# dsilvestro/LiteRate

Measured on AMD Instinct MI355X. Metric: RJMCMC iters/sec x lineages (lineage-log-lik evals/s, summed over chains), higher is better.
Workload: dtype f64

## Files before the change

### literate_amd/_hip.py

```python
import ctypes as C
import os

from .build import LIB

c_i32, c_i64, c_f64, c_vp = C.c_int32, C.c_int64, C.c_double, C.c_void_p

LR_ERR_NULL, LR_ERR_SIZE, LR_ERR_MODEL, LR_ERR_WORKSPACE, LR_ERR_T0, LR_ERR_STATE, LR_ERR_ORDER = -1, -2, -3, -4, -5, -6, -7
ERRORS = {-1: "LR_ERR_NULL", -2: "LR_ERR_SIZE", -3: "LR_ERR_MODEL", -4: "LR_ERR_WORKSPACE", -5: "LR_ERR_T0",
          -6: "LR_ERR_STATE", -7: "LR_ERR_ORDER (lineages must be sorted by birth time for the persistent engines)"}

LR_KMAX, LR_ROW, LR_MAX_BINS = 32, 64, 4094
LR_WARN_KCAP = 2
LR_STATE_ROWS, LR_ISTATE_ROWS = 9, 5
LR_TRACE_HEAD = 13
LR_TRACE_W = LR_TRACE_HEAD + 2 * (2 * LR_KMAX - 1)
LR_SIMBATCH_GROUPS, LR_SIMBATCH_LDS_SLOTS = 512, 16384
LR_SHIFT_PRIOR_KCAP, LR_SHIFT_PRIOR_BLOCKS = 64, 768
LR_ESS_LDS_ROWS = 16384
ROW_L, ROW_M, ROW_TL, ROW_TM, ROW_PL, ROW_PM, ROW_PTL, ROW_PTM, ROW_SCALARS = range(9)
(S_LIKA, S_PRIORA, S_PRIORPOIA, S_GRATE_L, S_GRATE_M, S_POI, S_HASTING, S_PRIOR_P, S_PRIORPOI_P, S_CONST_P,
 S_CONST_A, S_LIK_P, S_LOG_G0, S_LOG_G1, S_LOG_POI) = range(15)
IROW_EL, IROW_EM, IROW_PEL, IROW_PEM, IROW_SCALARS = range(5)
(I_KL, I_KM, I_PKL, I_PKM, I_GIBBS, I_INVALID, I_IT_LO, I_IT_HI, I_ACCEPTED, I_MOVE, I_NEXT_LO, I_NEXT_HI,
 I_SLOT) = range(13)


class McmcConfig(C.Structure):
    _fields_ = [("n_lineages", c_i64), ("n_bins", c_i32), ("n_chains", c_i32), ("model", c_i32),
                ("const_rates", c_i32), ("const_death_rate", c_i32), ("use_rate_HP", c_i32), ("s_freq", c_i32),
                ("n_trace_slots", c_i32), ("poisson_HP", c_f64), ("update_fraction", c_f64), ("t0", c_f64),
# ... 60 lines not shown
    "lr_curve_summary": (c_i32, [c_vp, c_i32, c_i32, c_i32, c_i32, c_i32, c_i32, c_i32, c_vp, c_i32, c_f64, c_i32, c_vp,
                                 c_vp, c_i64, c_vp]),
    "lr_mcmc_query_layout": (c_i32, [C.POINTER(McmcConfig), C.POINTER(McmcLayout)]),
    "lr_mcmc_create": (c_i32, [C.POINTER(McmcConfig), c_vp, c_vp, c_vp, c_vp, c_i64, C.POINTER(c_vp)]),
    "lr_mcmc_init": (c_i32, [c_vp, c_vp, c_vp, c_vp, c_vp, c_vp, c_vp, c_i32, c_vp]),
    "lr_mcmc_steps": (c_i32, [c_vp, c_i64, c_vp]),
    "lr_mcmc_time_scan": (c_i32, [c_vp, c_i32, C.POINTER(C.c_float), c_vp]),
    "lr_mcmc_time_steps": (c_i32, [c_vp, c_i64, C.POINTER(C.c_float), c_vp]),
    "lr_mcmc_restore": (c_i32, [c_vp, c_vp]),
    "lr_mcmc_describe": (c_i32, [c_vp, C.c_char_p, c_i32]),
    "lr_mcmc_status": (c_i32, [c_vp, C.POINTER(c_i32), c_vp]),
    "lr_mcmc_warnings": (c_i32, [c_vp, C.POINTER(c_i32), c_vp]),
    "lr_mcmc_destroy": (c_i32, [c_vp]),
    "lr_debug_draws": (c_i32, [C.c_uint64, c_i64, c_vp, c_vp, c_vp, c_vp, c_vp, c_i32, c_vp, c_vp]),
    "lr_debug_stream2": (c_i32, [c_vp, c_vp, c_i64, c_vp, c_vp]),
}

_lib = None


class HipLibraryError(RuntimeError):
    pass


def load():
    global _lib
    if _lib is not None:
        return _lib
    if not os.path.exists(LIB):
        raise HipLibraryError("libliterate_hip.so not found at %s - run `python -m literate_amd.build` "
# ... 38 lines not shown
```

### literate_amd/build.py

```python
import json
import os
import shutil
import subprocess
from concurrent.futures import ThreadPoolExecutor

HERE = os.path.dirname(os.path.abspath(__file__))
CSRC = os.path.join(HERE, "csrc")
LIB = os.path.join(CSRC, "libliterate_hip.so")
BUILD_INFO = os.path.join(CSRC, "libliterate_hip.build.json")
OBJ_DIR = os.path.join(CSRC, "_build")
SOURCES = ["lr_stats.hip", "lr_loglik.hip", "lr_mcmc.hip", "lr_spec.hip", "lr_stream.hip", "lr_packscan.hip", "lr_pack.hip", "lr_sim.hip", "lr_simbatch.hip", "lr_format.hip", "lr_summary.hip", "lr_prior.hip", "lr_ess.hip", "lr_curves.hip", "lr_waic.hip", "lr_loo.hip"]
HEADERS = ["lr_device.h", "lr_math.h", "lr_chain.h", "lr_dd.h", "lr_scan.h", "lr_step.h", "lr_spec.h", "lr_engine.h", "lr_internal.h",
           os.path.join("..", "..", "include", "literate_hip.h")]
TU_FLAGS = {"lr_spec.hip": os.environ.get("LR_SPEC_FLAGS", "-mllvm -disable-machine-licm").split(),
            "lr_mcmc.hip": os.environ.get("LR_MCMC_FLAGS", "-mllvm -disable-machine-licm").split(),
            "lr_stream.hip": os.environ.get("LR_STREAM_FLAGS", "-mllvm -disable-machine-licm").split()}
ASYNC_UNITS = {"lr_mcmc.hip": 60, "lr_spec.hip": 0, "lr_packscan.hip": 16}


def _stale():
    if not os.path.exists(LIB):
        return True
    t = os.path.getmtime(LIB)
    return any(os.path.getmtime(os.path.join(CSRC, f)) > t for f in SOURCES + HEADERS)


# ... 72 lines not shown
```

### literate_amd/csrc/lr_engine.h

```cpp
#pragma once
#include "lr_internal.h"
#include "lr_scan.h"
#include "lr_step.h"

#define LR_MAX_PARTS 4
struct lr_part {
    int base, count, hA;
    bool pipelined;
    hipStream_t stream;
    hipEvent_t done;
    hipGraphExec_t graph_exec;
    int graph_units;
};

struct lr_p4_shares {
    int delta[16];
    int n_slots;
    int help_trips;
};

struct lr_engine {
    lr_mcmc_config cfg;
    lr_mcmc_layout lay;
    lr_scan_plan plan;
// ... 14 lines not shown
    hipEvent_t fork;
    hipEvent_t ev0, ev1;
};


#define LR_P4_MAX_GIVE 64
#define LR_IDX_SPARE ((LR_P4_MAX_GIVE + 2) * 1024)
#define LR_MAX_RUNS (1ll << 20)

static inline long long lr_groups_alloc(long long n_lineages) {
    const long long runs = n_lineages < LR_MAX_RUNS ? n_lineages : LR_MAX_RUNS;
    return (n_lineages + LR_SLOTS - 1) / LR_SLOTS + runs + LR_IDX_SPARE;
}

#define LR_P4_CARRY_BYTES 512

#define LR_H_WIDE 520

#ifndef LR_SPEC_THREADS
#define LR_SPEC_THREADS 768
#endif
#ifndef LR_SPEC_THREADS_SINGLE
#define LR_SPEC_THREADS_SINGLE 768
#endif
#ifndef LR_SPEC_SCAN_UNROLL
#define LR_SPEC_SCAN_UNROLL 1
#endif
#ifndef LR_SPEC_SCAN_PRIO
#define LR_SPEC_SCAN_PRIO 2
#endif
// ... 43 lines not shown
```

### literate_amd/csrc/lr_mcmc.hip

```cpp
#include <cmath>
#include <cstdio>
#include <cstdlib>
#include <new>

#include "lr_chain.h"
#include "lr_dd.h"
#include "lr_engine.h"
#include "lr_internal.h"
#include "lr_scan.h"
#include "lr_step.h"

__global__ __launch_bounds__(LR_WAVE) void lr_rj_propose_score_kernel(
    const double* __restrict__ rates, const double* __restrict__ times, const int* __restrict__ K, int kmax,
    const int* __restrict__ move, const int* __restrict__ index, const double* __restrict__ draws, double mult_d,
    double* __restrict__ out_rates, double* __restrict__ out_times, int* __restrict__ out_K,
    double* __restrict__ out_score) {
    const int c = blockIdx.x, lane = threadIdx.x;
    int k = K[c];
    double R = (lane < k) ? rates[(size_t)c * kmax + lane] : 0.0;
    double T = (lane <= k) ? times[(size_t)c * (kmax + 1) + lane] : 0.0;
    const double* dr = draws + (size_t)c * 2 * kmax;
    const int mv = move[c];
    double score = 0.0;
    if (mv == 0) {
// ... 146 lines not shown
    lr_persist_scan<H, GENERAL>(reinterpret_cast<const char*>(tab), pk, g0, g1 - g0, tid, 256, &acc0, &acc1);
    const double s0 = lr_wave_sum(acc0), s1 = lr_wave_sum(acc1);
    if (lane == 0) red[wave][0] = s0, red[wave][1] = s1;
    __syncthreads();
    if (tid < 2 && 2 * pair + tid < n_chains)
        partials[(size_t)(2 * pair + tid) * lr_tile_stride(tiles) + tile] = ((red[0][tid] + red[1][tid]) + red[2][tid]) + red[3][tid];
}

typedef __attribute__((address_space(3))) double lr_lds_f64;
typedef __attribute__((address_space(3))) int lr_lds_i32;
template <int PB, int ES, bool PRE = false, int SAMPLER = -1, bool HAND = false>
__device__ __forceinline__ void lr_persist_step_body(const __attribute__((address_space(3))) lr_step_args* a3, int c, int lane,
                                                     __attribute__((address_space(3))) lr_seg_scratch* scratch3,
                                                     lr_lds_f64* st_f64, lr_lds_i32* st_i32, double lik, lr_lds_f64* table3,
                                                     lr_lds_f64* br3 ,
                                                     const lr_draw_slot* draws = nullptr ,
                                                     lr_table_hand* hand = nullptr, int hand_epoch = 0) {
    constexpr int table_es = ES;
    const lr_step_args& a = *(const lr_step_args*)a3;
    const double* br_lds = (const double*)br3;
    LR_SSTAMP(0);
    lr_chain_regs st;
    lr_chain_load(st, (double*)st_f64, (int*)st_i32, lane);
    if (SAMPLER == 1 || (SAMPLER == -1 && a.cfg.sampler != 0))
        lr_dd_step_core<true>(st, a, 0, c, lane, lik, reinterpret_cast<double2*>((double*)table3), table_es, br_lds);
    else if (PRE) {
        lr_rj_draws pre;
        lr_draws_load(draws, pre, lane);
        lr_chain_step_core<true, PB, HAND>(st, a, 0, c, lane, (lr_seg_scratch*)scratch3, lik, reinterpret_cast<double2*>((double*)table3),
                                           table_es, br_lds, br_lds + LR_H_WIDE, &pre, hand, hand_epoch);
    } else
        lr_chain_step_core<true, PB>(st, a, 0, c, lane, (lr_seg_scratch*)scratch3, lik, reinterpret_cast<double2*>((double*)table3),
                                     table_es, br_lds, br_lds + LR_H_WIDE);
    if (HAND) lr_chain_store_handed(st, (double*)st_f64, (int*)st_i32, lane);
    else lr_chain_store(st, (double*)st_f64, (int*)st_i32, lane);
    LR_SSTAMP(8);
}

template <int NA>
__device__ __forceinline__ void lr_p4_leave_sums(double2 (*part)[LR_WAVE], int* arrived, double* out, int slot, int lane,
                                                 int& scans_done, double s0, double s1) {
    part[slot][lane] = make_double2(s0, s1);
    int prev = 0;
// ... 15 lines not shown

template <int PB, int ES>
__device__ __attribute__((noinline)) void lr_persist_step(const __attribute__((address_space(3))) lr_step_args* a3, int c, int lane,
                                                          __attribute__((address_space(3))) lr_seg_scratch* scratch3,
                                                          lr_lds_f64* st_f64, lr_lds_i32* st_i32, double lik, lr_lds_f64* table3,
                                                          lr_lds_f64* br3) {
    lr_persist_step_body<PB, ES>(a3, c, lane, scratch3, st_f64, st_i32, lik, table3, br3);
}

template <int PB, int ES, int NW, int SAMPLER, bool HELP>
__device__ __attribute__((noinline)) void lr_persist4_steppers(const __attribute__((address_space(3))) lr_step_args* a3, int c0,
                                                               int n_chains, int wave, int lane,
                                                               __attribute__((address_space(3))) lr_seg_scratch* scratch3,
                                                               lr_lds_f64* st_f64, lr_lds_i32* st_i32, lr_lds_f64* red,
                                                               lr_lds_f64* tab, int tab_doubles, lr_lds_f64* br3, long long n_iters,
                                                               const lr_draw_slot* draws ,
                                                               lr_table_hand* hands ) {
    static_assert(!HELP || (ES == 2 && SAMPLER == 0), "helper waves: RJ sampler at unit resolution");
    for (long long iter = 0; iter < n_iters; ++iter) {
#pragma unroll 1
        for (int ph = 0; ph < 2; ++ph) {
#ifdef LR_DIAG
            const unsigned long long dq0 = wall_clock64();
#endif
            const int c = c0 + 2 * ph + wave;
            if (c < n_chains) {
                double lik = 0.0;
#pragma unroll
                for (int w2 = 2; w2 < (ES == 2  ? 3 : NW); ++w2) lik += red[(ph * NW + w2) * 2 + wave];
                lr_persist_step_body<PB, ES, ES == 2  && SAMPLER == 0, SAMPLER, HELP>(
                    a3, c, lane, scratch3, st_f64 + (2 * ph + wave) * (LR_STATE_ROWS * LR_ROW),
                    st_i32 + (2 * ph + wave) * (LR_ISTATE_ROWS * LR_ROW), lik, tab + ph * tab_doubles + wave, br3,
                    draws + (2 * ph + wave), HELP ? hands + wave : nullptr, (int)((2 * iter + ph + 1) & 0x3fffffff));
            }
#ifdef LR_DIAG
            const unsigned long long dq1 = wall_clock64();
#endif
            __syncthreads();
#ifdef LR_DIAG
            if (lane == 0 && blockIdx.x < 64) {
                atomicAdd(&lr_diag_step[16384 + (blockIdx.x * 16 + wave) * 4 + 0], dq1 - dq0);
                atomicAdd(&lr_diag_step[16384 + (blockIdx.x * 16 + wave) * 4 + 1], wall_clock64() - dq1);
            }
#endif
        }
    }
}

// ... 131 lines not shown
}

#ifndef LR_P4_THREADS
#define LR_P4_THREADS 1024
#endif
#ifdef LR_DIAG
#define LR_PSTAMP(k) if (threadIdx.x == 0 && blockIdx.x < 64) lr_diag_step[28672 + blockIdx.x * 8 + (k)] = wall_clock64()
#else
#define LR_PSTAMP(k)
#endif

template <int H, bool GENERAL, bool PARAM ,
          bool HELP = false>
__global__ __launch_bounds__(LR_P4_THREADS, LR_P4_THREADS / 256) void lr_persist4_kernel(const lr_step_args* __restrict__ ap ,
                                                                       lr_packed_lineages pk, long long n8,
                                                                       lr_p4_shares sh, long long n_iters, char* carry_all) {
    static_assert(!HELP || (!GENERAL && !PARAM), "helper waves: RJ sampler at unit resolution");
    const lr_step_args& a = *ap;
    LR_PSTAMP(0);
    constexpr int NW = LR_P4_THREADS / LR_WAVE;
    constexpr int W0 = HELP ? 4 : 2;
    constexpr int NS = NW - W0;
    constexpr int LR_P4_SCANNERS = NS * LR_WAVE;
    constexpr int ENT = GENERAL ? 2 : 1;
    constexpr int ES = GENERAL ? 6 * H : 2;
    __shared__ double2 tab[2][LR_UNIT_PLANES * H];
    __shared__ double red[2][NW][2];
    constexpr bool LAST_SUMS = !GENERAL;
    __shared__ double2 part[LAST_SUMS ? NW - 2 : 1][LR_WAVE];
    __shared__ int arrived;
    __shared__ lr_table_hand hands[2];
    __shared__ lr_seg_scratch scratch[2];
    __shared__ double st_f64[4][LR_STATE_ROWS * LR_ROW];
    __shared__ int st_i32[4][LR_ISTATE_ROWS * LR_ROW];
    __shared__ lr_step_args a_lds;
    __shared__ double br_lds[2][LR_H_WIDE];
    __shared__ lr_draw_slot draws_s[4];
    lr_draw_slot* const draws = draws_s;
    const int tid = threadIdx.x, lane = tid & (LR_WAVE - 1), wave = tid / LR_WAVE;
    if (tid < (int)(sizeof(lr_step_args) / 4)) reinterpret_cast<int*>(&a_lds)[tid] = reinterpret_cast<const int*>(ap)[tid];
    for (int b = tid; b < LR_H_WIDE; b += blockDim.x) {
        const bool in = b < ap->cfg.n_bins;
        br_lds[0][b] = (in && ap->br_length) ? ap->br_length[b] : 0.0;
        br_lds[1][b] = in ? ap->log_br[b] : 0.0;
    }
    constexpr bool draw_ahead = !GENERAL && !PARAM;
    auto draw_duty = [&](int pr) {
        const int q = wave - W0, k = q & 1, ch = 2 * pr + k;
        if (!draw_ahead || q < 0 || q >= (HELP ? 2 : 4) || (int)(blockIdx.x * 4) + ch >= ap->cfg.n_chains) return;
        const int* I = st_i32[ch] + LR_IROW_SCALARS * LR_ROW;
        const unsigned long long it = ((unsigned long long)(unsigned int)I[LR_I_IT_HI] << 32 | (unsigned int)I[LR_I_IT_LO]) + 1ull;
        lr_draw_slot* slot = &draws[ch];
        if (HELP) lr_spec_draw_both(a_lds, (int)(blockIdx.x * 4) + ch, lane, it, slot);
        else lr_spec_draw_part(a_lds, (int)(blockIdx.x * 4) + ch, lane, it, slot, q >> 1);
    };
    auto help_duty = [&](int ph, int epoch) {
        const int k = wave - 2;
        const int ch = 2 * ph + k;
        if ((int)(blockIdx.x * 4) + ch >= ap->cfg.n_chains) return;
        lr_table_hand* hand = &hands[k];
#ifdef LR_DIAG
        const unsigned long long dh0 = wall_clock64();
#endif
        while (__hip_atomic_load(&hand->epoch, __ATOMIC_RELAXED, __HIP_MEMORY_SCOPE_WORKGROUP) != epoch) __builtin_amdgcn_s_sleep(1);
        asm volatile("" ::: "memory");
#ifdef LR_DIAG
        if (lane == 0 && blockIdx.x < 64) atomicAdd(&lr_diag_step[16384 + (blockIdx.x * 16 + wave) * 4 + 2], wall_clock64() - dh0);
#endif
        const lr_seg_scratch* sc = &scratch[k];
        const int eL = lane <= LR_KMAX ? sc->edge[0][lane] : 0, eM = lane <= LR_KMAX ? sc->edge[1][lane] : 0;
// ... 15 lines not shown
            lr_p4_leave_sums<NA>(part, &arrived, &red[pr][2][0], wave >= W0 ? wave - W0 : NS + wave - 2, lane, scans_done, s0, s1);
        } else {
            s0 = lr_wave_sum(s0), s1 = lr_wave_sum(s1);
            if (lane == 0) red[pr][wave][0] = s0, red[pr][wave][1] = s1;
        }
    };
    const int c0 = blockIdx.x * 4;
    const int C = a.cfg.n_chains;
    if (wave < 4 && c0 + wave < C) {
        const int c = c0 + wave;
        const double* S = a.state_f64 + (size_t)c * LR_STATE_ROWS * LR_ROW;
        const int* I = a.state_i32 + (size_t)c * LR_ISTATE_ROWS * LR_ROW;
        for (int r = 0; r < LR_STATE_ROWS; ++r) st_f64[wave][r * LR_ROW + lane] = S[r * LR_ROW + lane];
        for (int r = 0; r < LR_ISTATE_ROWS; ++r) st_i32[wave][r * LR_ROW + lane] = I[r * LR_ROW + lane];
    }
    double2* g0 = lr_chain_table(a, c0);
    double2* g1 = lr_chain_table(a, c0 + 2);
    for (int i = tid; i < 2 * H * ENT; i += LR_P4_THREADS) {
        const int e = GENERAL ? lr_pairgen_lds_entry(i, H) : i;
        tab[0][e] = g0[i], tab[1][e] = g1[i];
    }
    __syncthreads();
    LR_PSTAMP(1);
    if (GENERAL) {
        lr_pair_planes_block_general(tab[0], H, a.cfg.n_bins, tid, LR_P4_THREADS);
        lr_pair_planes_block_general(tab[1], H, a.cfg.n_bins, tid, LR_P4_THREADS);
    } else {
        lr_pair_planes_block(tab[0], H, a.cfg.n_bins, tid, LR_P4_THREADS);
        lr_pair_planes_block(tab[1], H, a.cfg.n_bins, tid, LR_P4_THREADS);
    }
// ... 6 lines not shown
    const int k_tot = (int)((n8 - nh_ + LR_P4_SCANNERS - 1) / LR_P4_SCANNERS);
    const int k_mine = k_tot + (scanner ? sh.delta[wave - W0] : 0);
    bool any_shift = false;
#pragma unroll
    for (int q = 0; q < NS; ++q) any_shift |= sh.delta[q] != 0;
    const long long nh = HELP ? (long long)sh.help_trips * (2 * LR_WAVE) : 0;
    const long long n8w = any_shift ? (long long)k_mine * LR_P4_SCANNERS : n8 - nh;
    auto help_scan = [&](int pr) {
        double s0 = 0.0, s1 = 0.0;
        if (nh > 0) lr_persist_scan<H, GENERAL, 1, false, false>(reinterpret_cast<const char*>(tab[pr]), pk, 0, nh, tid - 2 * LR_WAVE, 2 * LR_WAVE, &s0, &s1);
        leave_sums(pr, s0, s1);
    };
    static_assert(2 * NW * 8 + 4 <= LR_P4_CARRY_BYTES, "");
    char* carry = carry_all ? carry_all + (size_t)blockIdx.x * LR_P4_CARRY_BYTES : nullptr;
    const bool carried = carry && *reinterpret_cast<const int*>(carry + 2 * NW * 8) == 1;
    auto prologue_draws = [&]() { draw_duty(0); };
    if (carried) {
        if (tid < 2 * NW) (&red[0][0][0])[tid] = reinterpret_cast<const double*>(carry)[tid];
        if (scanner) prologue_draws();
    } else if (scanner) {
        double s0 = 0.0, s1 = 0.0;
        lr_scan_tail tail;
        lr_persist_scan<H, GENERAL, 1, false, true>(reinterpret_cast<const char*>(tab[0]), pk, nh, n8w, sid, LR_P4_SCANNERS, &s0, &s1, nullptr, &tail);
        leave_sums(0, s0, s1);
        lr_scan_drain(tail);
        prologue_draws();
    }
    if (helper && !carried) help_scan(0);
    __syncthreads();
    LR_PSTAMP(3);
    if (helper) {
        for (long long iter = 0; iter < n_iters; ++iter) {
#pragma unroll 1
            for (int ph = 0; ph < 2; ++ph) {
#ifdef LR_DIAG
                const unsigned long long dq0 = wall_clock64();
#endif
                help_scan(1 - ph);
                help_duty(ph, (int)((2 * iter + ph + 1) & 0x3fffffff));
#ifdef LR_DIAG
                const unsigned long long dq1 = wall_clock64();
#endif
                __syncthreads();
#ifdef LR_DIAG
                if (lane == 0 && blockIdx.x < 64) {
                    atomicAdd(&lr_diag_step[16384 + (blockIdx.x * 16 + wave) * 4 + 0], dq1 - dq0);
                    atomicAdd(&lr_diag_step[16384 + (blockIdx.x * 16 + wave) * 4 + 1], wall_clock64() - dq1);
                }
#endif
            }
        }
    } else if (!scanner)
        lr_persist4_steppers<(H <= 264 ? lr_bins_per_lane(H) : 0), ES, NW, PARAM ? 1 : 0, HELP>(
            (const __attribute__((address_space(3))) lr_step_args*)&a_lds, c0, C, wave, lane,
            (__attribute__((address_space(3))) lr_seg_scratch*)&scratch[wave], (lr_lds_f64*)&st_f64[0][0], (lr_lds_i32*)&st_i32[0][0],
            (lr_lds_f64*)&red[0][0][0], (lr_lds_f64*)reinterpret_cast<double*>(tab[0]), 2 * LR_UNIT_PLANES * H,
            (lr_lds_f64*)&br_lds[0][0], n_iters, &draws[0], &hands[0]);
    else
    for (long long iter = 0; iter < n_iters; ++iter) {
#pragma unroll
        for (int ph = 0; ph < 2; ++ph) {
#ifdef LR_DIAG
            const unsigned long long dq0 = wall_clock64();
#endif
            {
                double s0 = 0.0, s1 = 0.0;
                lr_scan_tail tail;
                lr_persist_scan<H, GENERAL, 1, false, true>(reinterpret_cast<const char*>(tab[1 - ph]), pk, nh, n8w, sid, LR_P4_SCANNERS, &s0, &s1, nullptr, &tail);
                leave_sums(1 - ph, s0, s1);
                lr_scan_drain(tail);
                draw_duty(1 - ph);
            }
#ifdef LR_DIAG
            const unsigned long long dq1 = wall_clock64();
#endif
            __syncthreads();
#ifdef LR_DIAG
            if (lane == 0 && blockIdx.x < 64) {
                atomicAdd(&lr_diag_step[16384 + (blockIdx.x * 16 + wave) * 4 + 0], dq1 - dq0);
                atomicAdd(&lr_diag_step[16384 + (blockIdx.x * 16 + wave) * 4 + 1], wall_clock64() - dq1);
            }
#endif
        }
    }
    LR_PSTAMP(4);
    if (wave < 4 && c0 + wave < C) {
// ... 399 lines not shown
    out->pack_tmp = o, o += lr_align_up64(lr_pack_tmp_bytes(cfg->n_lineages), 256);
    out->args_blob = o, o += 1024;
    out->tables = o, o += lr_align_up64((long long)lr_align_up64(C, p.cb < 2 ? 2 : p.cb) * p.tab_stride * 16, 256);
    out->partials = o, o += lr_align_up64((long long)lr_tile_stride(p.tiles) * C * 8, 256);
    out->trace = o, o += lr_align_up64((long long)cfg->n_trace_slots * C * LR_TRACE_W * 8, 256);
    int team_k = 0, team_cpb = 0;
    out->persistent = lr_persist_variant(cfg, p, &team_k, &team_cpb);
    out->spec_chains_per_team = team_cpb;
    {
        int base[LR_MAX_PARTS + 1], hA[LR_MAX_PARTS];
        bool pipelined[LR_MAX_PARTS];
        const bool packed = lr_packscan_planned(cfg, p);
        const int parts = lr_partition(cfg->n_chains, p.cb, lr_fused_supported(p), base, hA, pipelined, lr_packed_mode(cfg, p));
        out->packed_scan = (out->persistent == 0 && packed) ? 1 : 0;
        out->streaming = (out->persistent == 0 && !out->packed_scan && parts == 1 && !pipelined[0] && lr_stream_eligible(cfg, p)) ? 1 : 0;
        out->reserved3 = 0;
    }
    if (p.unit == LR_TAB_PAIRGEN && out->persistent == 0 && !lr_packscan_planned(cfg, p)) return LR_ERR_STATE;
    out->team_blocks = team_k;
    out->table_mode = p.unit;
    out->status = o, o += 256;
    out->xchg = o, o += (team_k > 1) ? lr_align_up64(2ll * C * LR_TEAM_MAX * LR_SPEC_GRANULES * 8, 256)
                                     : (out->persistent == 2 ? lr_align_up64((C + 3) / 4 * LR_P4_CARRY_BYTES, 256)
                                        : (out->streaming ? LR_STREAM_SYNC_BYTES + lr_align_up64((long long)lr_align_up64(C, p.cb < 2 ? 2 : p.cb) * p.tab_stride * 16, 256) : 0));
    out->total_bytes = o;
    out->table_stride = p.tab_stride;
    out->tiles = p.tiles;
    out->chains_per_block = p.cb;
    out->trace_width = LR_TRACE_W;
    {
        int base[LR_MAX_PARTS + 1], hA[LR_MAX_PARTS];
        bool pipelined[LR_MAX_PARTS];
        out->n_parts = lr_partition(cfg->n_chains, p.cb, lr_fused_supported(p), base, hA, pipelined, lr_packed_mode(cfg, p));
        out->pipelined = pipelined[0] ? 1 : 0;
    }
    {
        static const int wide_env = lr_env_int("LR_PERSIST_WIDE", -1);
        const bool wide = wide_env >= 0 ? wide_env != 0 : ((cfg->n_chains + 1) / 2 <= 256 && cfg->n_lineages >= 20000);
        out->reserved1 = out->persistent == 3 ? (team_cpb == 1 ? LR_SPEC_THREADS_SINGLE : LR_SPEC_THREADS) : (out->persistent == 2 ? 1024 : (out->persistent == 1 ? (wide ? 1024 : 512) : 0));
// ... 327 lines not shown
    hipStream_t stream = (hipStream_t)stream_;
    const lr_step_args a = lr_make_args(e);
    if (e->persistent) {
        const uint4* idx8 = (const uint4*)(e->ws + e->lay.lineage_idx);
        const bool general = e->plan.unit == LR_TAB_PAIRGEN;
        lr_packed_lineages pk;
        pk.idx8 = idx8, pk.frac = general ? (const uint4*)(e->ws + e->lay.lineage_frac) : nullptr, pk.fstride = e->n8_alloc;
        if (e->n8 <= 0) return LR_ERR_STATE;
        const lr_step_args* ap = (const lr_step_args*)(e->ws + e->lay.args_blob);
        const int blocks = (e->cfg.n_chains + 1) / 2;
        const bool p4 = e->lay.persistent == 2;
        const bool param = e->cfg.sampler != 0;
        static const int prio = lr_env_int("LR_PERSIST_PRIO", 12);
        const bool wide = e->lay.reserved1 == 1024;
        if (e->lay.persistent == 3) return lr_launch_spec(e, a, pk, n_iters, stream);
        for (int64_t done = 0; done < n_iters;) {
            const int64_t n = (n_iters - done > 4096) ? 4096 : n_iters - done;
        static const int carry_env = lr_env_int("LR_P4_CARRY", 1);
        char* p4_carry = (p4 && carry_env) ? e->ws + e->lay.xchg : nullptr;
#define LR_P_LAUNCH(HH)                                                                                                       \
    if (p4) {                                                                                                                 \
        const dim3 g4((e->cfg.n_chains + 3) / 4), b4(LR_P4_THREADS);                                                          \
        if (general && param) hipLaunchKernelGGL((lr_persist4_kernel<HH, true, true>), g4, b4, 0, stream, ap, pk, e->n8, e->p4, (long long)n, p4_carry);   \
        else if (general) hipLaunchKernelGGL((lr_persist4_kernel<HH, true, false>), g4, b4, 0, stream, ap, pk, e->n8, e->p4, (long long)n, p4_carry);      \
        else if (param) hipLaunchKernelGGL((lr_persist4_kernel<HH, false, true>), g4, b4, 0, stream, ap, pk, e->n8, e->p4, (long long)n, p4_carry);        \
        else if (e->p4_help)                                                 \
            hipLaunchKernelGGL((lr_persist4_kernel<(HH <= 264 ? HH : 264), false, false, true>), g4, b4, 0, stream, ap, pk, e->n8, e->p4, (long long)n, p4_carry); \
        else hipLaunchKernelGGL((lr_persist4_kernel<HH, false, false>), g4, b4, 0, stream, ap, pk, e->n8, e->p4, (long long)n, p4_carry);                  \
    } else if (wide) {                                                                                                        \
        hipLaunchKernelGGL((lr_persist_kernel<HH, 1024>), dim3(blocks), dim3(1024), 0, stream, ap, idx8, e->n8, e->p4, (long long)n, 0); \
    } else {                                                                                                                  \
        hipLaunchKernelGGL((lr_persist_kernel<HH, 512>), dim3(blocks), dim3(512), 0, stream, ap, idx8, e->n8, e->p4, (long long)n, prio); \
    }
            switch (e->plan.H) {
                case 40: LR_P_LAUNCH(40); break;
                case 72: LR_P_LAUNCH(72); break;
                case 136: LR_P_LAUNCH(136); break;
                case 264: LR_P_LAUNCH(264); break;
                default: LR_P_LAUNCH(LR_H_WIDE); break;
            }
#undef LR_P_LAUNCH
            const int rc = (int)hipGetLastError();
            if (rc) return rc;
// ... 127 lines not shown
```

### literate_amd/csrc/lr_step.h

```cpp
#pragma once
#include "lr_chain.h"
#include "lr_dd.h"
#include "lr_internal.h"
#include "lr_scan.h"

struct lr_step_args {
    lr_mcmc_config cfg;
    double* state_f64;
    int* state_i32;
    const double* log_br;
    double2* tables;
    const double* partials;
    double* trace;
    const double* br_length;
    double log_T;
    double mult_l;
    const double* dd_consts;
    int tab_stride, n_cls, tiles, H, unit, cb;
    unsigned int* warn;
};

__device__ __forceinline__ double2* lr_chain_table(const lr_step_args& a, int c) {
    if (!a.unit) return a.tables + (size_t)c * a.tab_stride;
    if (a.unit == LR_TAB_PAIRGEN)
// ... 494 lines not shown
    double beta = 0.0;
    if (!(r_a < 0.8) && r_a < 0.999 && cfg.const_rates == 0 && q_b > 0.5) {
        double ga, gb;
        lr_wave_gamma2(rng, it, LR_P_BETA_A, LR_SHAPE_BETA_RJ, LR_P_BETA_B, LR_SHAPE_BETA_RJ, lane, &ga, &gb);
        beta = ga / (ga + gb);
    }
    double so = lr_bcast(lu, LR_UD_LANE);
    so = (lane == 1) ? r_a : so;
    so = (lane == 2) ? lr_bcast(u.b, LR_UD_LANE + 1) : so;
    so = (lane == 3) ? lr_bcast(u.a, LR_UD_LANE + 2) : so;
    so = (lane == 4) ? q_b : so;
    so = (lane == 5) ? lr_bcast(u.a, LR_UD_LANE + 3) : so;
    so = (lane == 6) ? lr_bcast(u.b, LR_UD_LANE + 3) : so;
    so = (lane == 7) ? beta : so;
    if (lane < 8) out->sc[lane] = so;
}

struct lr_table_hand {
    int epoch;
    int KL, KM;
    int reuse;
    int noop;
    int out_idx, base_idx;
    int pad_;
    double par[8];
};

template <bool LDS_CONSTS = false, int PB = 0, int CS = 2, bool PAIR_PLANES = true, bool HAND = false>
__device__ __forceinline__ void lr_propose_rj(const lr_step_args& a, int c, int lane, lr_seg_scratch* scratch_p,
                                              uint64_t it, lr_rj_state& s, lr_rj_prop& p, double2* table,
// ... 529 lines not shown
```

### literate_amd/engine.py

```python
import ctypes as C
import hashlib
import os
from collections import namedtuple

import numpy as np

from . import _hip, ops


class ChainEngine:
    def __init__(self, ts, te, n_chains, model=0, seed=1, const_rates=0, const_death_rate=0, use_rate_HP=1,
                 poisson_HP=0.0, update_fraction=0.75, s_freq=1000, n_trace_slots=0, chain_offset=0,
                 device=None, stats=None, sort_lineages=True, unit_resolution=None, engine="auto", dd=None, team=0,
                 chains_per_team=0):
        torch = _hip.require_gpu()
        self.lib = _hip.load()
        self.device = torch.device(device or "cuda")
        ts_d = ops._dev(ts, torch.float64, self.device)
        te_d = ops._dev(te, torch.float64, self.device)
        if sort_lineages:
            o1 = torch.sort(te_d, stable=True).indices
            o2 = torch.sort(torch.floor(ts_d[o1]), stable=True).indices
            order = o1[o2]
            ts_d, te_d = ts_d[order].contiguous(), te_d[order].contiguous()
# ... 213 lines not shown
    _CFG_KEYS = ("n_lineages", "n_bins", "n_chains", "model", "const_rates", "const_death_rate", "use_rate_HP",
                 "s_freq", "n_trace_slots", "poisson_HP", "update_fraction", "t0", "start_time", "end_time", "seed",
                 "chain_offset", "unit_resolution", "frac_birth", "frac_death", "sampler", "m_birth", "m_death",
                 "dd_present", "dd_init_death", "engine_mode")

    def _signature(self):
        sig = {k: repr(getattr(self.cfg, k)) for k in self._CFG_KEYS}
        sig.update({"layout_" + f: repr(getattr(self.layout, f)) for f, _ in self.layout._fields_})
        sig["data_sha1"] = self._data_hash
        sig["format"] = "2: state in .npz (head, tail), trace rows in .npz.trace"
        return sig

    def _trace_span(self):
        return int(self.layout.trace), int(self.layout.status)

    def checkpoint_begin(self):
        import torch
        t0, t1 = self._trace_span()
        with torch.cuda.device(self.device):
            head, tail = self.workspace[:t0].clone(), self.workspace[t1:].clone()
            ev = torch.cuda.Event()
            ev.record()
        return dict(head=head, tail=tail, ev=ev, iterations=int(self.iterations), samples=int(self.samples_done()))

    def checkpoint_write(self, ticket, path):
        import torch
        path = str(path)
        if not path.endswith(".npz"):
            path += ".npz"
        side = getattr(self, "_ckpt_stream", None)
        if side is None:
            side = self._ckpt_stream = torch.cuda.Stream(device=self.device)
        row_bytes = self.n_chains * _hip.LR_TRACE_W * 8
        s1 = ticket["samples"]
        sidecar = path + ".trace"
# ... 33 lines not shown
        ticket = self.checkpoint_begin()
        self.check_status()
        self.checkpoint_write(ticket, path)

    def load(self, path):
        import torch
        path = str(path)
        with np.load(path) as z:
            saved = dict(zip([str(k) for k in z["sig_keys"]], [str(v) for v in z["sig_vals"]]))
            mine = self._signature()
            bad = [k for k in mine if k not in saved or mine[k] != saved[k]]
            if bad or len(saved) != len(mine):
                raise ValueError("checkpoint was written by a different configuration: " + ", ".join(bad))
            t0, t1 = self._trace_span()
            head, tail = torch.from_numpy(z["head"]), torch.from_numpy(z["tail"])
            if head.numel() != t0 or tail.numel() != self.workspace.numel() - t1:
                raise ValueError("checkpoint workspace size differs")
            n_rows = int(z["n_trace_rows"])
            row_bytes = self.n_chains * _hip.LR_TRACE_W * 8
            if n_rows > 0:
                sidecar = path + ".trace"
                if not os.path.exists(sidecar) or os.path.getsize(sidecar) < n_rows * row_bytes:
                    raise ValueError("checkpoint trace file %s is missing or shorter than the %d rows the checkpoint holds" % (sidecar, n_rows))
                rows = np.fromfile(sidecar, dtype=np.uint8, count=n_rows * row_bytes)
                self.workspace[t0:t0 + n_rows * row_bytes].copy_(torch.from_numpy(rows).to(self.device))
            self.workspace[:t0].copy_(head.to(self.device))
            self.workspace[t1:].copy_(tail.to(self.device))
            self.iterations = int(z["iterations"])
        self._ckpt_saved = {path: n_rows}
        _hip.check(_hip.launch(self.lib.lr_mcmc_restore, self.device, self.handle), "lr_mcmc_restore")

    def close(self):
        if getattr(self, "handle", None) is not None:
            self.lib.lr_mcmc_destroy(self.handle)
            self.handle = None

    def __del__(self):
        try:
            self.close()
        except Exception:
            pass

# ... 119 lines not shown
```

Measured before the change: 16100 billion.

## Pre-draw RJ random numbers in a separate kernel before persistent4 chunks

Moves the per-iteration RJ draws out of the persistent4 kernel, where scanner/helper waves produced them into shared slots, into a separate predraw kernel. That kernel fills a global record buffer for a chunk of iterations and all chains. The persistent kernel then loads each chain's next record with a nontemporal vector load one phase ahead, which takes RNG work off the critical step path. The cost is extra workspace (up to about 1 GiB), an extra launch per chunk, and global memory traffic.

```diff
diff --git a/literate_amd/_hip.py b/literate_amd/_hip.py
--- a/literate_amd/_hip.py
+++ b/literate_amd/_hip.py
@@ -14,6 +14,7 @@
 LR_STATE_ROWS, LR_ISTATE_ROWS = 9, 5
 LR_TRACE_HEAD = 13
 LR_TRACE_W = LR_TRACE_HEAD + 2 * (2 * LR_KMAX - 1)
+LR_REC_DOUBLES = 128
 LR_SIMBATCH_GROUPS, LR_SIMBATCH_LDS_SLOTS = 512, 16384
 LR_SHIFT_PRIOR_KCAP, LR_SHIFT_PRIOR_BLOCKS = 64, 768
 LR_ESS_LDS_ROWS = 16384
@@ -104,6 +105,7 @@
     "lr_mcmc_destroy": (c_i32, [c_vp]),
     "lr_debug_draws": (c_i32, [C.c_uint64, c_i64, c_vp, c_vp, c_vp, c_vp, c_vp, c_i32, c_vp, c_vp]),
     "lr_debug_stream2": (c_i32, [c_vp, c_vp, c_i64, c_vp, c_vp]),
+    "lr_debug_rj_draws": (c_i32, [C.POINTER(McmcConfig), c_i32, c_i32, C.c_uint64, c_i32, c_vp, c_vp, c_vp]),
 }
 
 _lib = None
diff --git a/literate_amd/build.py b/literate_amd/build.py
--- a/literate_amd/build.py
+++ b/literate_amd/build.py
@@ -9,7 +9,7 @@
 LIB = os.path.join(CSRC, "libliterate_hip.so")
 BUILD_INFO = os.path.join(CSRC, "libliterate_hip.build.json")
 OBJ_DIR = os.path.join(CSRC, "_build")
-SOURCES = ["lr_stats.hip", "lr_loglik.hip", "lr_mcmc.hip", "lr_spec.hip", "lr_stream.hip", "lr_packscan.hip", "lr_pack.hip", "lr_sim.hip", "lr_simbatch.hip", "lr_format.hip", "lr_summary.hip", "lr_prior.hip", "lr_ess.hip", "lr_curves.hip", "lr_waic.hip", "lr_loo.hip"]
+SOURCES = ["lr_stats.hip", "lr_loglik.hip", "lr_mcmc.hip", "lr_predraw.hip", "lr_spec.hip", "lr_stream.hip", "lr_packscan.hip", "lr_pack.hip", "lr_sim.hip", "lr_simbatch.hip", "lr_format.hip", "lr_summary.hip", "lr_prior.hip", "lr_ess.hip", "lr_curves.hip", "lr_waic.hip", "lr_loo.hip"]
 HEADERS = ["lr_device.h", "lr_math.h", "lr_chain.h", "lr_dd.h", "lr_scan.h", "lr_step.h", "lr_spec.h", "lr_engine.h", "lr_internal.h",
            os.path.join("..", "..", "include", "literate_hip.h")]
 TU_FLAGS = {"lr_spec.hip": os.environ.get("LR_SPEC_FLAGS", "-mllvm -disable-machine-licm").split(),
diff --git a/literate_amd/csrc/lr_engine.h b/literate_amd/csrc/lr_engine.h
--- a/literate_amd/csrc/lr_engine.h
+++ b/literate_amd/csrc/lr_engine.h
@@ -52,6 +52,24 @@
 }
 
 #define LR_P4_CARRY_BYTES 512
+
+static inline int lr_p4_rec_chains(int n_chains) { return (n_chains + 3) / 4 * 4; }
+static inline int lr_p4_draw_chunk_default(int persistent, int table_mode, const lr_mcmc_config* cfg) {
+    if (persistent != 2 || table_mode == LR_TAB_PAIRGEN || cfg->sampler != 0) return 0;
+    const long long b = (1ll << 30) / ((long long)lr_p4_rec_chains(cfg->n_chains) * (LR_REC_DOUBLES * 8));
+    return b > 4096 ? 4096 : (b < 1 ? 1 : (int)b);
+}
+static inline int lr_p4_draw_chunk(const lr_engine* e) {
+    static const char* env = getenv("LR_P4_DRAW_CHUNK");
+    const int v = env ? atoi(env) : 0;
+    return (v >= 1 && v < e->lay.reserved3) ? v : e->lay.reserved3;
+}
+static inline long long lr_p4_recs_offset(const lr_engine* e) {
+    return e->lay.xchg + lr_align_up64((long long)(e->cfg.n_chains + 3) / 4 * LR_P4_CARRY_BYTES, 256);
+}
+int lr_launch_predraw(uint64_t seed, int64_t chain_offset, int const_rates, double mult_l, const int* state_i32,
+                      unsigned long long it_first, int chain_first, int n_chains, int n_iters, int rec_cq, double* recs,
+                      hipStream_t stream);
 
 #define LR_H_WIDE 520
 
diff --git a/literate_amd/csrc/lr_mcmc.hip b/literate_amd/csrc/lr_mcmc.hip
--- a/literate_amd/csrc/lr_mcmc.hip
+++ b/literate_amd/csrc/lr_mcmc.hip
@@ -184,7 +184,7 @@
                                                      __attribute__((address_space(3))) lr_seg_scratch* scratch3,
                                                      lr_lds_f64* st_f64, lr_lds_i32* st_i32, double lik, lr_lds_f64* table3,
                                                      lr_lds_f64* br3 ,
-                                                     const lr_draw_slot* draws = nullptr ,
+                                                     lr_f64x2 rec = lr_f64x2{0.0, 0.0} ,
                                                      lr_table_hand* hand = nullptr, int hand_epoch = 0) {
     constexpr int table_es = ES;
     const lr_step_args& a = *(const lr_step_args*)a3;
@@ -196,7 +196,7 @@
         lr_dd_step_core<true>(st, a, 0, c, lane, lik, reinterpret_cast<double2*>((double*)table3), table_es, br_lds);
     else if (PRE) {
         lr_rj_draws pre;
-        lr_draws_load(draws, pre, lane);
+        lr_draws_from_rec(rec, pre, lane);
         lr_chain_step_core<true, PB, HAND>(st, a, 0, c, lane, (lr_seg_scratch*)scratch3, lik, reinterpret_cast<double2*>((double*)table3),
                                            table_es, br_lds, br_lds + LR_H_WIDE, &pre, hand, hand_epoch);
     } else
@@ -242,9 +242,11 @@
                                                                __attribute__((address_space(3))) lr_seg_scratch* scratch3,
                                                                lr_lds_f64* st_f64, lr_lds_i32* st_i32, lr_lds_f64* red,
                                                                lr_lds_f64* tab, int tab_doubles, lr_lds_f64* br3, long long n_iters,
-                                                               const lr_draw_slot* draws ,
+                                                               const double* recs, int rec_cq, lr_f64x2 rec0,
                                                                lr_table_hand* hands ) {
     static_assert(!HELP || (ES == 2 && SAMPLER == 0), "helper waves: RJ sampler at unit resolution");
+    constexpr bool PRE = ES == 2  && SAMPLER == 0;
+    lr_f64x2 rec = rec0;
     for (long long iter = 0; iter < n_iters; ++iter) {
 #pragma unroll 1
         for (int ph = 0; ph < 2; ++ph) {
@@ -256,10 +258,14 @@
                 double lik = 0.0;
 #pragma unroll
                 for (int w2 = 2; w2 < (ES == 2  ? 3 : NW); ++w2) lik += red[(ph * NW + w2) * 2 + wave];
-                lr_persist_step_body<PB, ES, ES == 2  && SAMPLER == 0, SAMPLER, HELP>(
+                lr_persist_step_body<PB, ES, PRE, SAMPLER, HELP>(
                     a3, c, lane, scratch3, st_f64 + (2 * ph + wave) * (LR_STATE_ROWS * LR_ROW),
                     st_i32 + (2 * ph + wave) * (LR_ISTATE_ROWS * LR_ROW), lik, tab + ph * tab_doubles + wave, br3,
-                    draws + (2 * ph + wave), HELP ? hands + wave : nullptr, (int)((2 * iter + ph + 1) & 0x3fffffff));
+                    rec, HELP ? hands + wave : nullptr, (int)((2 * iter + ph + 1) & 0x3fffffff));
+            }
+            if (PRE) {
+                const int cn = c0 + 2 * (1 - ph) + wave;
+                if (iter + ph < n_iters && cn < n_chains) rec = lr_rec_load(recs, iter + ph, rec_cq, cn, lane);
             }
 #ifdef LR_DIAG
             const unsigned long long dq1 = wall_clock64();
@@ -421,7 +427,8 @@
           bool HELP = false>
 __global__ __launch_bounds__(LR_P4_THREADS, LR_P4_THREADS / 256) void lr_persist4_kernel(const lr_step_args* __restrict__ ap ,
                                                                        lr_packed_lineages pk, long long n8,
-                                                                       lr_p4_shares sh, long long n_iters, char* carry_all) {
+                                                                       lr_p4_shares sh, long long n_iters, char* carry_all,
+                                                                       const double* __restrict__ recs , int rec_cq) {
     static_assert(!HELP || (!GENERAL && !PARAM), "helper waves: RJ sampler at unit resolution");
     const lr_step_args& a = *ap;
     LR_PSTAMP(0);
@@ -442,8 +449,6 @@
     __shared__ int st_i32[4][LR_ISTATE_ROWS * LR_ROW];
     __shared__ lr_step_args a_lds;
     __shared__ double br_lds[2][LR_H_WIDE];
-    __shared__ lr_draw_slot draws_s[4];
-    lr_draw_slot* const draws = draws_s;
     const int tid = threadIdx.x, lane = tid & (LR_WAVE - 1), wave = tid / LR_WAVE;
     if (tid < (int)(sizeof(lr_step_args) / 4)) reinterpret_cast<int*>(&a_lds)[tid] = reinterpret_cast<const int*>(ap)[tid];
     for (int b = tid; b < LR_H_WIDE; b += blockDim.x) {
@@ -452,15 +457,6 @@
         br_lds[1][b] = in ? ap->log_br[b] : 0.0;
     }
     constexpr bool draw_ahead = !GENERAL && !PARAM;
-    auto draw_duty = [&](int pr) {
-        const int q = wave - W0, k = q & 1, ch = 2 * pr + k;
-        if (!draw_ahead || q < 0 || q >= (HELP ? 2 : 4) || (int)(blockIdx.x * 4) + ch >= ap->cfg.n_chains) return;
-        const int* I = st_i32[ch] + LR_IROW_SCALARS * LR_ROW;
-        const unsigned long long it = ((unsigned long long)(unsigned int)I[LR_I_IT_HI] << 32 | (unsigned int)I[LR_I_IT_LO]) + 1ull;
-        lr_draw_slot* slot = &draws[ch];
-        if (HELP) lr_spec_draw_both(a_lds, (int)(blockIdx.x * 4) + ch, lane, it, slot);
-        else lr_spec_draw_part(a_lds, (int)(blockIdx.x * 4) + ch, lane, it, slot, q >> 1);
-    };
     auto help_duty = [&](int ph, int epoch) {
         const int k = wave - 2;
         const int ch = 2 * ph + k;
@@ -506,6 +502,8 @@
         for (int r = 0; r < LR_STATE_ROWS; ++r) st_f64[wave][r * LR_ROW + lane] = S[r * LR_ROW + lane];
         for (int r = 0; r < LR_ISTATE_ROWS; ++r) st_i32[wave][r * LR_ROW + lane] = I[r * LR_ROW + lane];
     }
+    lr_f64x2 rec0 = lr_f64x2{0.0, 0.0};
+    if (draw_ahead && wave < 2 && c0 + wave < C && n_iters > 0) rec0 = lr_rec_load(recs, 0, rec_cq, c0 + wave, lane);
     double2* g0 = lr_chain_table(a, c0);
     double2* g1 = lr_chain_table(a, c0 + 2);
     for (int i = tid; i < 2 * H * ENT; i += LR_P4_THREADS) {
@@ -542,17 +540,14 @@
     static_assert(2 * NW * 8 + 4 <= LR_P4_CARRY_BYTES, "");
     char* carry = carry_all ? carry_all + (size_t)blockIdx.x * LR_P4_CARRY_BYTES : nullptr;
     const bool carried = carry && *reinterpret_cast<const int*>(carry + 2 * NW * 8) == 1;
-    auto prologue_draws = [&]() { draw_duty(0); };
     if (carried) {
         if (tid < 2 * NW) (&red[0][0][0])[tid] = reinterpret_cast<const double*>(carry)[tid];
-        if (scanner) prologue_draws();
     } else if (scanner) {
         double s0 = 0.0, s1 = 0.0;
         lr_scan_tail tail;
         lr_persist_scan<H, GENERAL, 1, false, true>(reinterpret_cast<const char*>(tab[0]), pk, nh, n8w, sid, LR_P4_SCANNERS, &s0, &s1, nullptr, &tail);
         leave_sums(0, s0, s1);
         lr_scan_drain(tail);
-        prologue_draws();
     }
     if (helper && !carried) help_scan(0);
     __syncthreads();
@@ -583,7 +578,7 @@
             (const __attribute__((address_space(3))) lr_step_args*)&a_lds, c0, C, wave, lane,
             (__attribute__((address_space(3))) lr_seg_scratch*)&scratch[wave], (lr_lds_f64*)&st_f64[0][0], (lr_lds_i32*)&st_i32[0][0],
             (lr_lds_f64*)&red[0][0][0], (lr_lds_f64*)reinterpret_cast<double*>(tab[0]), 2 * LR_UNIT_PLANES * H,
-            (lr_lds_f64*)&br_lds[0][0], n_iters, &draws[0], &hands[0]);
+            (lr_lds_f64*)&br_lds[0][0], n_iters, recs, rec_cq, rec0, &hands[0]);
     else
     for (long long iter = 0; iter < n_iters; ++iter) {
 #pragma unroll
@@ -597,7 +592,6 @@
                 lr_persist_scan<H, GENERAL, 1, false, true>(reinterpret_cast<const char*>(tab[1 - ph]), pk, nh, n8w, sid, LR_P4_SCANNERS, &s0, &s1, nullptr, &tail);
                 leave_sums(1 - ph, s0, s1);
                 lr_scan_drain(tail);
-                draw_duty(1 - ph);
             }
 #ifdef LR_DIAG
             const unsigned long long dq1 = wall_clock64();
@@ -1027,7 +1021,6 @@
         const int parts = lr_partition(cfg->n_chains, p.cb, lr_fused_supported(p), base, hA, pipelined, lr_packed_mode(cfg, p));
         out->packed_scan = (out->persistent == 0 && packed) ? 1 : 0;
         out->streaming = (out->persistent == 0 && !out->packed_scan && parts == 1 && !pipelined[0] && lr_stream_eligible(cfg, p)) ? 1 : 0;
-        out->reserved3 = 0;
     }
     if (p.unit == LR_TAB_PAIRGEN && out->persistent == 0 && !lr_packscan_planned(cfg, p)) return LR_ERR_STATE;
     out->team_blocks = team_k;
@@ -1036,6 +1029,8 @@
     out->xchg = o, o += (team_k > 1) ? lr_align_up64(2ll * C * LR_TEAM_MAX * LR_SPEC_GRANULES * 8, 256)
                                      : (out->persistent == 2 ? lr_align_up64((C + 3) / 4 * LR_P4_CARRY_BYTES, 256)
                                         : (out->streaming ? LR_STREAM_SYNC_BYTES + lr_align_up64((long long)lr_align_up64(C, p.cb < 2 ? 2 : p.cb) * p.tab_stride * 16, 256) : 0));
+    out->reserved3 = lr_p4_draw_chunk_default(out->persistent, p.unit, cfg);
+    o += (long long)out->reserved3 * lr_p4_rec_chains(cfg->n_chains) * (LR_REC_DOUBLES * 8);
     out->total_bytes = o;
     out->table_stride = p.tab_stride;
     out->tiles = p.tiles;
@@ -1393,19 +1388,27 @@
         static const int prio = lr_env_int("LR_PERSIST_PRIO", 12);
         const bool wide = e->lay.reserved1 == 1024;
         if (e->lay.persistent == 3) return lr_launch_spec(e, a, pk, n_iters, stream);
+        const int rec_cq = lr_p4_rec_chains(e->cfg.n_chains);
+        const int64_t cut = e->lay.reserved3 > 0 ? lr_p4_draw_chunk(e) : 4096;
+        double* recs = e->lay.reserved3 > 0 ? (double*)(e->ws + lr_p4_recs_offset(e)) : nullptr;
         for (int64_t done = 0; done < n_iters;) {
-            const int64_t n = (n_iters - done > 4096) ? 4096 : n_iters - done;
+            const int64_t n = (n_iters - done > cut) ? cut : n_iters - done;
+            if (recs) {
+                const int rcd = lr_launch_predraw(e->cfg.seed, e->cfg.chain_offset, e->cfg.const_rates, a.mult_l,
+                                                  (const int*)(e->ws + e->lay.state_i32), 0ull, 0, e->cfg.n_chains, (int)n, rec_cq, recs, stream);
+                if (rcd) return rcd;
+            }
         static const int carry_env = lr_env_int("LR_P4_CARRY", 1);
         char* p4_carry = (p4 && carry_env) ? e->ws + e->lay.xchg : nullptr;
 #define LR_P_LAUNCH(HH)                                                                                                       \
     if (p4) {                                                                                                                 \
         const dim3 g4((e->cfg.n_chains + 3) / 4), b4(LR_P4_THREADS);                                                          \
-        if (general && param) hipLaunchKernelGGL((lr_persist4_kernel<HH, true, true>), g4, b4, 0, stream, ap, pk, e->n8, e->p4, (long long)n, p4_carry);   \
-        else if (general) hipLaunchKernelGGL((lr_persist4_kernel<HH, true, false>), g4, b4, 0, stream, ap, pk, e->n8, e->p4, (long long)n, p4_carry);      \
-        else if (param) hipLaunchKernelGGL((lr_persist4_kernel<HH, false, true>), g4, b4, 0, stream, ap, pk, e->n8, e->p4, (long long)n, p4_carry);        \
+        if (general && param) hipLaunchKernelGGL((lr_persist4_kernel<HH, true, true>), g4, b4, 0, stream, ap, pk, e->n8, e->p4, (long long)n, p4_carry, recs, rec_cq);   \
+        else if (general) hipLaunchKernelGGL((lr_persist4_kernel<HH, true, false>), g4, b4, 0, stream, ap, pk, e->n8, e->p4, (long long)n, p4_carry, recs, rec_cq);      \
+        else if (param) hipLaunchKernelGGL((lr_persist4_kernel<HH, false, true>), g4, b4, 0, stream, ap, pk, e->n8, e->p4, (long long)n, p4_carry, recs, rec_cq);        \
         else if (e->p4_help)                                                 \
-            hipLaunchKernelGGL((lr_persist4_kernel<(HH <= 264 ? HH : 264), false, false, true>), g4, b4, 0, stream, ap, pk, e->n8, e->p4, (long long)n, p4_carry); \
-        else hipLaunchKernelGGL((lr_persist4_kernel<HH, false, false>), g4, b4, 0, stream, ap, pk, e->n8, e->p4, (long long)n, p4_carry);                  \
+            hipLaunchKernelGGL((lr_persist4_kernel<(HH <= 264 ? HH : 264), false, false, true>), g4, b4, 0, stream, ap, pk, e->n8, e->p4, (long long)n, p4_carry, recs, rec_cq); \
+        else hipLaunchKernelGGL((lr_persist4_kernel<HH, false, false>), g4, b4, 0, stream, ap, pk, e->n8, e->p4, (long long)n, p4_carry, recs, rec_cq);                  \
     } else if (wide) {                                                                                                        \
         hipLaunchKernelGGL((lr_persist_kernel<HH, 1024>), dim3(blocks), dim3(1024), 0, stream, ap, idx8, e->n8, e->p4, (long long)n, 0); \
     } else {                                                                                                                  \
diff --git a/literate_amd/csrc/lr_predraw.hip b/literate_amd/csrc/lr_predraw.hip
--- /dev/null
+++ b/literate_amd/csrc/lr_predraw.hip
@@ -0,0 +1,116 @@
+#include <cmath>
+
+#include "lr_engine.h"
+#include "lr_step.h"
+
+#define LR_PREDRAW_ITEMS 16
+#define LR_PREDRAW_WAVES 4
+
+__global__ __launch_bounds__(LR_PREDRAW_WAVES* LR_WAVE) void lr_predraw_kernel(uint32_t seed, uint32_t chain_offset, int const_rates, double mult_l,
+                                                                               const int* __restrict__ state_i32,
+                                                                               unsigned long long it_first, int chain_first, int n_chains,
+                                                                               long long n_items, int rec_cq, double* __restrict__ recs) {
+    const int lane = threadIdx.x & (LR_WAVE - 1), wave = threadIdx.x / LR_WAVE;
+    const long long base = ((long long)blockIdx.x * LR_PREDRAW_WAVES + wave) * LR_PREDRAW_ITEMS;
+    if (base >= n_items) return;
+    auto item = [&](long long i, int* c, long long* j, unsigned long long* it) {
+        *j = i / n_chains;
+        *c = chain_first + (int)(i - *j * n_chains);
+        unsigned long long t = it_first;
+        if (state_i32) {
+            const int* I = state_i32 + ((size_t)*c * LR_ISTATE_ROWS + LR_IROW_SCALARS) * LR_ROW;
+            t = ((unsigned long long)(unsigned int)I[LR_I_IT_HI] << 32 | (unsigned int)I[LR_I_IT_LO]) + 1ull;
+        }
+        *it = t + (unsigned long long)*j;
+    };
+    auto rec_of = [&](int c, long long j) { return recs + lr_rec_index(j, rec_cq, c - chain_first) * 2; };
+#pragma unroll 1
+    for (int p = 0; p < LR_PREDRAW_ITEMS / 2; ++p) {
+        const long long i = base + 2 * p + (lane >> 5);
+        const bool valid = i < n_items;
+        int c;
+        long long j;
+        unsigned long long it;
+        item(valid ? i : n_items - 1, &c, &j, &it);
+        const lr_stream rng{seed, chain_offset + (uint32_t)c};
+        const int idx = lane & 31;
+        const lr_u2 u = lr_pair(rng, it, LR_P_MULT, (uint32_t)idx);
+        const double x = mult_l * (u.b - .5);
+        const double m = exp(x);
+        if (valid) {
+            double* r = rec_of(c, j);
+            *reinterpret_cast<lr_f64x2*>(r + 2 * idx) = lr_f64x2{x, m};
+            r[2 * (32 + idx)] = u.a;
+        }
+    }
+    const int k_mine = lane >> 2, ul = lane & 3;
+    const long long i = base + k_mine;
+    const bool valid = i < n_items;
+    int c;
+    long long j;
+    unsigned long long it;
+    item(valid ? i : n_items - 1, &c, &j, &it);
+    const lr_stream rng{seed, chain_offset + (uint32_t)c};
+    const uint32_t purpose = (ul == 0) ? LR_P_ACCEPT : (ul == 1 ? LR_P_MOVE : LR_P_RJ);
+    const lr_u2 u = lr_pair(rng, it, purpose, ul == 3 ? 1u : 0u);
+    const double lu = lr_log(ul == 0 ? u.a : 1.0);
+    const double r_a = __shfl(u.a, (lane & ~3) + 1), q_b = __shfl(u.b, (lane & ~3) + 2);
+    const bool need = valid && ul == 0 && !(r_a < 0.8) && r_a < 0.999 && const_rates == 0 && q_b > 0.5;
+    double beta = 0.0;
+    for (unsigned long long todo = __ballot(need); todo != 0ull; todo &= todo - 1ull) {
+        const int src = __ffsll((long long)todo) - 1;
+        int ck;
+        long long jk;
+        unsigned long long itk;
+        item(base + (src >> 2), &ck, &jk, &itk);
+        const lr_stream rk{seed, chain_offset + (uint32_t)ck};
+        double ga, gb;
+        lr_wave_gamma2(rk, itk, LR_P_BETA_A, LR_SHAPE_BETA_RJ, LR_P_BETA_B, LR_SHAPE_BETA_RJ, lane, &ga, &gb);
+        const double bk = ga / (ga + gb);
+        if (lane == src) beta = bk;
+    }
+    if (valid) {
+        double* sc = rec_of(c, j) + 2 * 32 + 1;
+        if (ul == 0) sc[0] = lu, sc[2 * 7] = beta;
+        else sc[2 * (2 * ul - 1)] = u.a, sc[2 * (2 * ul)] = u.b;
+    }
+}
+
+__global__ __launch_bounds__(LR_WAVE) void lr_predraw_ref_kernel(lr_step_args a, unsigned long long it_first, int chain_first, int n_chains,
+                                                                 double* __restrict__ recs) {
+    __shared__ lr_draw_slot slot;
+    const int lane = threadIdx.x;
+    const long long j = blockIdx.x / n_chains;
+    const int c = chain_first + (int)(blockIdx.x - j * n_chains);
+    lr_spec_draw_both(a, c, lane, it_first + (unsigned long long)j, &slot);
+    __syncthreads();
+    lr_rec_store_slot(recs + lr_rec_index(j, n_chains, c - chain_first) * 2, &slot, lane);
+}
+
+int lr_launch_predraw(uint64_t seed, int64_t chain_offset, int const_rates, double mult_l, const int* state_i32,
+                      unsigned long long it_first, int chain_first, int n_chains, int n_iters, int rec_cq, double* recs,
+                      hipStream_t stream) {
+    const long long n_items = (long long)n_iters * n_chains;
+    const long long per_block = LR_PREDRAW_ITEMS * LR_PREDRAW_WAVES;
+    const long long blocks = (n_items + per_block - 1) / per_block;
+    if (blocks < 1 || blocks > 0x7fffffffll) return LR_ERR_SIZE;
+    hipLaunchKernelGGL(lr_predraw_kernel, dim3((unsigned)blocks), dim3(LR_PREDRAW_WAVES * LR_WAVE), 0, stream, (uint32_t)seed,
+                       (uint32_t)chain_offset, const_rates, mult_l, state_i32, it_first, chain_first, n_chains, n_items, rec_cq, recs);
+    return (int)hipGetLastError();
+}
+
+extern "C" int lr_debug_rj_draws(const lr_mcmc_config* cfg, int32_t chain_first, int32_t n_chains, uint64_t it_first,
+                                 int32_t n_iters, double* out_gen, double* out_ref, void* stream_) {
+    if (!cfg || !out_gen || !out_ref) return LR_ERR_NULL;
+    if (chain_first < 0 || n_chains < 1 || n_iters < 1 || (long long)n_chains * n_iters > (1ll << 24)) return LR_ERR_SIZE;
+    hipStream_t stream = (hipStream_t)stream_;
+    lr_step_args a = {};
+    a.cfg = *cfg;
+    a.mult_l = 2.0 * log(LR_MULT_D);
+    int rc = lr_launch_predraw(cfg->seed, cfg->chain_offset, cfg->const_rates, a.mult_l, nullptr, it_first, chain_first, n_chains,
+                               n_iters, n_chains, out_gen, stream);
+    if (rc) return rc;
+    hipLaunchKernelGGL(lr_predraw_ref_kernel, dim3((unsigned)(n_chains * n_iters)), dim3(LR_WAVE), 0, stream, a, it_first,
+                       chain_first, n_chains, out_ref);
+    return (int)hipGetLastError();
+}
diff --git a/literate_amd/csrc/lr_step.h b/literate_amd/csrc/lr_step.h
--- a/literate_amd/csrc/lr_step.h
+++ b/literate_amd/csrc/lr_step.h
@@ -532,6 +532,27 @@
     so = (lane == 6) ? lr_bcast(u.b, LR_UD_LANE + 3) : so;
     so = (lane == 7) ? beta : so;
     if (lane < 8) out->sc[lane] = so;
+}
+
+#define LR_REC_DOUBLES 128
+typedef double lr_f64x2 __attribute__((ext_vector_type(2)));
+__device__ __forceinline__ size_t lr_rec_index(long long j, int cq, int c) { return ((size_t)j * cq + c) * (LR_REC_DOUBLES / 2); }
+__device__ __forceinline__ lr_f64x2 lr_rec_load(const double* recs, long long j, int cq, int c, int lane) {
+    typedef const __attribute__((address_space(1))) lr_f64x2* gptr;
+    return __builtin_nontemporal_load((gptr)(reinterpret_cast<const lr_f64x2*>(recs) + lr_rec_index(j, cq, c) + lane));
+}
+__device__ __forceinline__ void lr_draws_from_rec(lr_f64x2 rec, lr_rj_draws& d, int lane) {
+    const double lo = rec.x, hi = rec.y;
+    d.x = lo, d.m = hi;
+    d.da = lr_half_hi(lo);
+    d.log_u = lr_bcast(hi, 32), d.r_a = lr_bcast(hi, 33), d.r_b = lr_bcast(hi, 34), d.q_a = lr_bcast(hi, 35);
+    d.q_b = lr_bcast(hi, 36), d.q2_a = lr_bcast(hi, 37), d.q2_b = lr_bcast(hi, 38), d.beta = lr_bcast(hi, 39);
+    (void)lane;
+}
+__device__ __forceinline__ void lr_rec_store_slot(double* rec, const lr_draw_slot* q, int lane) {
+    if (lane < 32) rec[2 * lane] = q->x[lane], rec[2 * lane + 1] = q->m[lane];
+    else rec[2 * lane] = q->da[lane - 32];
+    if (lane >= 32 && lane < 40) rec[2 * lane + 1] = q->sc[lane - 32];
 }
 
 struct lr_table_hand {
diff --git a/literate_amd/engine.py b/literate_amd/engine.py
--- a/literate_amd/engine.py
+++ b/literate_amd/engine.py
@@ -251,11 +251,15 @@
     def _trace_span(self):
         return int(self.layout.trace), int(self.layout.status)
 
+    def _state_end(self):
+        rec = int(self.layout.reserved3) * ((self.n_chains + 3) // 4 * 4) * _hip.LR_REC_DOUBLES * 8
+        return int(self.layout.total_bytes) - rec
+
     def checkpoint_begin(self):
         import torch
         t0, t1 = self._trace_span()
         with torch.cuda.device(self.device):
-            head, tail = self.workspace[:t0].clone(), self.workspace[t1:].clone()
+            head, tail = self.workspace[:t0].clone(), self.workspace[t1:self._state_end()].clone()
             ev = torch.cuda.Event()
             ev.record()
         return dict(head=head, tail=tail, ev=ev, iterations=int(self.iterations), samples=int(self.samples_done()))
@@ -319,7 +323,7 @@
                 raise ValueError("checkpoint was written by a different configuration: " + ", ".join(bad))
             t0, t1 = self._trace_span()
             head, tail = torch.from_numpy(z["head"]), torch.from_numpy(z["tail"])
-            if head.numel() != t0 or tail.numel() != self.workspace.numel() - t1:
+            if head.numel() != t0 or tail.numel() != self._state_end() - t1:
                 raise ValueError("checkpoint workspace size differs")
             n_rows = int(z["n_trace_rows"])
             row_bytes = self.n_chains * _hip.LR_TRACE_W * 8
@@ -330,7 +334,7 @@
                 rows = np.fromfile(sidecar, dtype=np.uint8, count=n_rows * row_bytes)
                 self.workspace[t0:t0 + n_rows * row_bytes].copy_(torch.from_numpy(rows).to(self.device))
             self.workspace[:t0].copy_(head.to(self.device))
-            self.workspace[t1:].copy_(tail.to(self.device))
+            self.workspace[t1:self._state_end()].copy_(tail.to(self.device))
             self.iterations = int(z["iterations"])
         self._ckpt_saved = {path: n_rows}
         _hip.check(_hip.launch(self.lib.lr_mcmc_restore, self.device, self.handle), "lr_mcmc_restore")
diff --git a/scratch/exp_p4_draw_chunk.py b/scratch/exp_p4_draw_chunk.py
--- /dev/null
+++ b/scratch/exp_p4_draw_chunk.py
@@ -0,0 +1,20 @@
+import os, subprocess, sys
+if len(sys.argv) > 1 and sys.argv[1] != "--one":
+    for b in sys.argv[1:]:
+        env = dict(os.environ)
+        env.pop("LR_P4_DRAW_CHUNK", None)
+        if int(b) > 0:
+            env["LR_P4_DRAW_CHUNK"] = b
+        out = subprocess.run([sys.executable, __file__, "--one"], env=env, capture_output=True, text=True).stdout.strip().splitlines()
+        print("chunk %5s: %s" % (b if int(b) > 0 else "dflt", out[-1] if out else "failed"), flush=True)
+    sys.exit(0)
+sys.path.insert(0, os.path.dirname(os.path.dirname(os.path.abspath(__file__))))
+import torch
+from literate_amd import synth
+from literate_amd.engine import ChainEngine
+ts, te, _ = synth.make_lineages(100000, 128, 20, 0)
+eng = ChainEngine(ts, te, 1024, model=0, seed=1, s_freq=100, n_trace_slots=80, engine="persistent4")
+eng.init(); eng.steps(3000); torch.cuda.synchronize()
+n = 2000
+t = sorted(eng.timed_steps(n) / n * 1e3 for _ in range(3))
+print("%.3f us/iter (median of 3 calls of %d; %.3f - %.3f), region %d iterations" % (t[1], n, t[0], t[2], eng.layout.reserved3))
```

Result: slower. 15460 billion (-4.0%).
